# zhirui-gao/Curve-Gaussian

Hardware: AMD Instinct MI355X
Metric: Msplats rasterized/s (fwd+bwd) (higher is better)
Workload: dtype f32

## Files before the change

curve_gaussian_amd/csrc/render.hip:

```cpp
#include "kernels.h"
#include "p2_mfma.h"
#include "composite.h"

namespace cgs {

constexpr int BATCH = 256;
__device__ __forceinline__ float sat01(float x) { return __builtin_amdgcn_fmed3f(x, 0.f, 1.f); }
struct StepConsts {
    float big, cA;
};
__device__ __forceinline__ StepConsts step_consts() {
    StepConsts k;
    k.big = 0x1p100f;
    k.cA = -__uint_as_float(0x3b808080u) * 0x1p100f;
    asm volatile("" : "+v"(k.big), "+v"(k.cA));
    return k;
}
constexpr int SLOTS = 8;

struct BucketSort {
    const uint32_t* tile_count;
    const uint64_t* keys;
    uint32_t* point_list;
    uint2* ranges;
    uint32_t* total;
    uint32_t cap;
};

struct ViewEpilogue {
    float* color_clamped;
    float* dir_out;
    const float* wv;
};

constexpr int GROUP = 16;
#ifndef CGS_FWD3_WAVES
#define CGS_FWD3_WAVES 6
#endif
#ifndef CGS_FWD3_WAVES_GENERAL
#define CGS_FWD3_WAVES_GENERAL CGS_FWD3_WAVES
#endif
#ifndef CGS_FWD_FAST
#define CGS_FWD_FAST 1
#endif
#ifndef CGS_BWD3_WAVES
#define CGS_BWD3_WAVES 6
#endif
#ifndef CGS_BWD3_CAP
#define CGS_BWD3_CAP 104
#endif
constexpr int BWD_BATCH = 128;
static_assert(CGS_BWD3_CAP % 8 == 0 && CGS_BWD3_CAP <= BWD_BATCH, "CGS_BWD3_CAP: a multiple of SLOTS (8), at most BWD_BATCH");
constexpr uint32_t BWD_PAD_OFF = (BWD_BATCH + 1) * 16;
constexpr uint32_t PAD_OFF = (BATCH + 1) * 16;

template <bool GEO, bool SORT, bool UNIT = false, bool TAG = UNIT>
__global__ void __launch_bounds__(256, UNIT ? CGS_FWD3_WAVES : CGS_FWD3_WAVES_GENERAL) k_render_fwd3(const uint2* __restrict__ ranges,
                                                     const uint32_t* __restrict__ point_list, int W, int H, int grid_x,
                                                     const SplatRec* __restrict__ rec, float* __restrict__ final_T,
                                                     uint32_t* __restrict__ n_contrib, const float* __restrict__ bg_color,
                                                     float* __restrict__ out_color, float* __restrict__ out_invdepth,
                                                     float* __restrict__ out_all_map, BucketSort bs, ViewEpilogue epi) {
    constexpr bool IMAGE_ONLY = UNIT && !GEO;
    __shared__ float4 s_geo[BATCH + 2];
    __shared__ float4 s_at[BATCH + 2];
    __shared__ float4 s_c[GEO ? BATCH + 2 : 1];
    __shared__ uint64_t s_qmask[4][4];
    __shared__ __attribute__((aligned(16))) uint32_t s_list[4][BATCH + GROUP];
    __shared__ __attribute__((aligned(16))) uint32_t s_ord[SORT ? RANK_MAX + RANK_U : 1];
    __shared__ uint32_t s_si[SORT ? RANK_MAX : 1];
    __shared__ uint32_t s_hist[SORT ? RANK_NB : 1], s_start[SORT ? RANK_NB + 1 : 1], s_mm[8];
    if (threadIdx.x == 0) {
        s_geo[BATCH + 1] = make_float4(0.f, 0.f, 0.f, 0.f);
        s_at[BATCH + 1] = make_float4(0.f, 0.f, 0.f, L2_NEVER);
        if (GEO) s_c[GEO ? BATCH + 1 : 0] = make_float4(0.f, 0.f, 0.f, 0.f);
    }
    const TileGeom g = tile_geom(W, H, grid_x);
    const int lane = g.lane;
    const float X0 = (float)(g.tx * TILE), Y0 = (float)(g.ty * TILE);
    uint2 range;
    bool prestaged = false;
    if (SORT) {
        const uint32_t tid = threadIdx.x;
        const uint32_t base = g.tile * bs.cap;
        uint64_t key0 = ~0ull;
        if (CGS_FWD_FAST && tid < bs.cap) key0 = bs.keys[base + tid];
        const uint32_t cnt = bs.tile_count[g.tile];
        const uint32_t n = min(cnt, bs.cap);
        range = make_uint2(base, base + n);
        if (tid == 0) {
            bs.ranges[g.tile] = range;
            if (cnt) {
                uint32_t* part = bs.total + 4 + 2 * (g.tile % TOTAL_PARTS);
                atomicAdd(&part[0], n);
                atomicMax(&part[1], cnt);
                if (cnt > bs.cap) {
                    bs.total[2] = 1u;
                    atomicAdd(&bs.total[TOTAL_WORDS], 1u);
                }
            }
        }
        if (CGS_FWD_FAST && n > 0 && n <= (uint32_t)BATCH) {
            const bool has = tid < n;
            const uint32_t depth = has ? (uint32_t)(key0 >> 32) : ~0u;
            const uint32_t id = has ? (uint32_t)key0 : 0u;
            const SplatRec* r = rec + id;
            float4 ra = make_float4(0.f, 0.f, 1.f, 0.f), rb = make_float4(1.f, 0.f, 0.f, 0.f), rc = ra;
            float tau2 = -1.f;
            if (has) {
                ra = r->a;
                rb = r->b;
                if (GEO) rc = r->c;
                tau2 = r->d.z;
            }
            if (has) s_ord[tid] = depth;
            if (tid < 4u) s_ord[n + tid] = 0x7f800000u;
            s_si[tid] = 0u;
            __syncthreads();
            uint32_t lost = 0u;
            if (((uint32_t)__builtin_amdgcn_readfirstlane((int)tid) & ~63u) < n) {
                const uint32_t rk[1] = {rank_loop_f32(reinterpret_cast<const float*>(s_ord), n, __uint_as_float(depth))};
                if (has) {
                    float4 sa, sb;
                    stage_splat(ra, rb, sa, sb);
                    const uint32_t slot = rk[0] + 1u;
                    s_geo[slot] = sa;
                    s_at[slot] = make_float4(sb.z, sb.w, sb.x, __builtin_amdgcn_logf(sb.y));
                    if (GEO) s_c[GEO ? slot : 0] = UNIT ? make_float4(rc.x, rc.y, rc.z, sb.w) : rc;
                    const uint32_t qm = quadrant_mask(ra, rb, tau2, X0, Y0);
                    lost = atomicExch(&s_si[rk[0]], 0x100u | qm);
                    bs.point_list[base + rk[0]] = TAG ? (id | (qm << LIST_TAG_SHIFT)) : id;
                }
            }
            prestaged = !__syncthreads_or((int)lost);
        }
        if (n > 0 && !prestaged) {
            uint32_t rank[4], idx[4];
            tile_rank_sort<4>(bs.keys + base, n, RankScratch{s_ord, s_si, s_hist, s_start, s_mm}, rank, idx);
#pragma unroll
            for (int q = 0; q < 4; q++) {
                const uint32_t i = tid + 256u * q;
                if (i < n) {
                    s_ord[rank[q]] = idx[q];
                    if (!TAG || rank[q] >= (uint32_t)BATCH) bs.point_list[base + rank[q]] = idx[q];
                }
            }
            __syncthreads();
        }
    } else {
        range = ranges[g.tile];
    }
    const int total = (int)(range.y - range.x);
    const int rounds = (total + BATCH - 1) / BATCH;
    const StepConsts k = step_consts();
    float T_dead = 0.0f;
    float Tw = 1.0f;
    float cA = g.inside ? k.cA : -0x1p126f;
    uint32_t last_contributor = 0;
    float C = 0.f, Dacc = 0.f;
    float A0 = 0.f, A1 = 0.f, A2 = 0.f, A3 = 0.f;
    bool wave_done = ballot64(cA > -0x1p120f) == 0ull;
    const P2Frag pix = p2_pixel_operand(lane);
    const int row_splat = p2_row_splat(lane);
    const float hx = X0 + (float)((g.wave & 1) << 3) + 3.5f;
    const float hy = Y0 + (float)((g.wave >> 1) << 3) + 4.f * (float)p2_row_half(lane) + 1.5f;
    uint32_t* const list = s_list[g.wave];
    const char* const geo_bytes = reinterpret_cast<const char*>(s_geo);
    const char* const at_bytes = reinterpret_cast<const char*>(s_at);
    const char* const c_bytes = reinterpret_cast<const char*>(s_c);

    for (int i = 0; i < rounds; i++) {
        if (!prestaged) {
            if (!__syncthreads_or(!wave_done)) break;
            const int progress = i * BATCH + threadIdx.x;
            uint32_t qm = 0;
            if (progress < total) {
                const uint32_t id = SORT ? s_ord[progress] : point_list[range.x + progress];
                const SplatRec* r = rec + id;
                const float4 a = r->a, b = r->b;
                float4 sa, sb;
                stage_splat(a, b, sa, sb);
                s_geo[threadIdx.x + 1] = sa;
                s_at[threadIdx.x + 1] = make_float4(sb.z, sb.w, sb.x, __builtin_amdgcn_logf(sb.y));
                if (GEO) s_c[threadIdx.x + 1] = UNIT ? make_float4(r->c.x, r->c.y, r->c.z, sb.w) : r->c;
                qm = quadrant_mask(a, b, r->d.z, X0, Y0);
                if (TAG) const_cast<uint32_t*>(SORT ? bs.point_list : point_list)[range.x + progress] = id | (qm << LIST_TAG_SHIFT);
            }
#pragma unroll
            for (int q = 0; q < 4; q++) {
                const uint64_t bal = ballot64((qm >> q) & 1u);
                if (lane == 0) s_qmask[q][g.wave] = bal;
            }
            __syncthreads();
        }
        if (wave_done) continue;
        int n = 0;
#pragma unroll
        for (int c = 0; c < 4; c++) {
            const uint64_t m = prestaged ? ballot64((s_si[SORT ? c * 64 + lane : 0] >> g.wave) & 1u) : uniform64(s_qmask[g.wave][c]);
            if ((m >> lane) & 1ull) {
                const int pos = n + (int)__builtin_amdgcn_mbcnt_hi((uint32_t)(m >> 32), __builtin_amdgcn_mbcnt_lo((uint32_t)m, 0u));
                list[pos] = (uint32_t)((c * 64 + lane + 1) * 16);
            }
            n += __builtin_popcountll(m);
        }
        if (lane < GROUP) list[n + lane] = PAD_OFF;
        __builtin_amdgcn_fence(__ATOMIC_RELEASE, "wavefront");
        __builtin_amdgcn_wave_barrier();
        __builtin_amdgcn_fence(__ATOMIC_ACQUIRE, "wavefront");
        uint32_t last_off = 0;
        for (int g0 = 0; g0 < n; g0 += GROUP) {
            f32x16 P;
            {
                const uint32_t joff = list[g0 + row_splat];
                const float4 ge = *reinterpret_cast<const float4*>(geo_bytes + joff);
                const float2 cl = *reinterpret_cast<const float2*>(at_bytes + joff + 8);
                P = p2_mfma(p2_splat_operand(lane, ge.x, ge.y, ge.z, ge.w, cl.x, cl.y, hx, hy), pix);
            }
            const int cnt = min(GROUP, n - g0);
            uint4 w4 = make_uint4(0u, 0u, 0u, 0u);
#pragma unroll
            for (int s = 0; s < GROUP; s += 2) {
                if (s < cnt) {
                if ((s & 3) == 0) w4 = *reinterpret_cast<const uint4*>(list + g0 + s);
                const uint32_t j0 = (s & 2) ? w4.z : w4.x, j1 = (s & 2) ? w4.w : w4.y;
                float2 t0 = make_float2(0.f, 0.f), t1 = t0;
                if (!UNIT) {
                    t0 = *reinterpret_cast<const float2*>(at_bytes + j0);
                    t1 = *reinterpret_cast<const float2*>(at_bytes + j1);
                }
                float4 c0 = make_float4(0.f, 0.f, 0.f, 0.f), c1 = c0;
                if (GEO) {
                    c0 = *reinterpret_cast<const float4*>(c_bytes + j0);
                    c1 = *reinterpret_cast<const float4*>(c_bytes + j1);
                }
                const float al0 = fminf(0.99f, __builtin_amdgcn_exp2f(P[s]));
                const float al1 = fminf(0.99f, __builtin_amdgcn_exp2f(P[s + 1]));
                const float a0 = al0 * sat01(fmaf(al0, k.big, cA));
                const float a1 = al1 * sat01(fmaf(al1, k.big, cA));
                float wa = a0 * Tw;
                float T1 = fmaf(-Tw, a0, Tw);
                float wb = a1 * T1;
                float T2 = fmaf(-T1, a1, T1);
                if (__builtin_expect(ballot64(T2 < 0.0001f) != 0ull, 0)) {
                    const bool d0 = T1 < 0.0001f;
                    T_dead = d0 ? Tw : T_dead;
                    wa = d0 ? 0.f : wa;
                    T1 = d0 ? 1.0f : T1;
                    const float a1e = d0 ? 0.f : a1;
                    wb = a1e * T1;
                    T2 = fmaf(-T1, a1e, T1);
                    const bool d1 = T2 < 0.0001f;
                    T_dead = d1 ? T1 : T_dead;
                    wb = d1 ? 0.f : wb;
                    T2 = d1 ? 1.0f : T2;
                    cA = (d0 || d1) ? -0x1p126f : cA;
                    if (UNIT) last_off = d0 ? j0 : d1 ? j1 : last_off;
                }
                Tw = T2;
                if (!UNIT) C = fmaf(t0.x, wa, C);
                if (!IMAGE_ONLY) Dacc = fmaf(UNIT ? c0.w : t0.y, wa, Dacc);
                if (GEO) { A0 = fmaf(c0.x, wa, A0); A1 = fmaf(c0.y, wa, A1); A2 = fmaf(c0.z, wa, A2); if (!UNIT) A3 = fmaf(c0.w, wa, A3); }
                if (!UNIT) C = fmaf(t1.x, wb, C);
                if (!IMAGE_ONLY) Dacc = fmaf(UNIT ? c1.w : t1.y, wb, Dacc);
                if (GEO) { A0 = fmaf(c1.x, wb, A0); A1 = fmaf(c1.y, wb, A1); A2 = fmaf(c1.z, wb, A2); if (!UNIT) A3 = fmaf(c1.w, wb, A3); }
                if (!UNIT) {
                    last_off = max(min(last_off, j0), min(max(last_off, j0), __float_as_uint(wa)));
                    last_off = max(min(last_off, j1), min(max(last_off, j1), __float_as_uint(wb)));
                }
            }
            }
            if (ballot64(cA > -0x1p120f) == 0ull) {
                wave_done = true;
                break;
            }
        }
        if (last_off) last_contributor = (uint32_t)(i * BATCH) + (last_off >> 4) - (UNIT ? 1u : 0u);
    }
    const bool terminated = !(cA > -0x1p120f);
    if (UNIT && !terminated) last_contributor = (uint32_t)total;
    if (g.inside) {
        const size_t HW = (size_t)H * W;
        const float T = terminated ? T_dead : Tw;
        final_T[g.pix_id] = T;
        n_contrib[g.pix_id] = last_contributor | (terminated ? NCONTRIB_TERMINATED : 0u);
        if (UNIT) C = A3 = 1.f - T;
        const float Cout = C + T * bg_color[0];
        out_color[g.pix_id] = Cout;
        if (SORT && epi.color_clamped) epi.color_clamped[g.pix_id] = fminf(fmaxf(Cout, 0.f), 1.f);
        if (SORT && GEO && epi.dir_out) {
            const float* wv = epi.wv;
            epi.dir_out[g.pix_id] = A0 * wv[0] + A1 * wv[1] + A2 * wv[2];
            epi.dir_out[HW + g.pix_id] = A0 * wv[4] + A1 * wv[5] + A2 * wv[6];
            epi.dir_out[2 * HW + g.pix_id] = A0 * wv[8] + A1 * wv[9] + A2 * wv[10];
        }
        if (!IMAGE_ONLY) out_invdepth[g.pix_id] = Dacc;
        if (IMAGE_ONLY) {
        } else if (GEO) {
            out_all_map[g.pix_id] = A0;
            out_all_map[HW + g.pix_id] = A1;
            out_all_map[2 * HW + g.pix_id] = A2;
            out_all_map[3 * HW + g.pix_id] = A3;
        } else {
            out_all_map[g.pix_id] = 0.f;
            out_all_map[HW + g.pix_id] = 0.f;
            out_all_map[2 * HW + g.pix_id] = 0.f;
            out_all_map[3 * HW + g.pix_id] = 0.f;
        }
    }
}

__device__ __forceinline__ float rows_sum(float v) {
    const unsigned x = __float_as_uint(v);
    auto s16 = __builtin_amdgcn_permlane16_swap(x, x, false, false);
    const float t = __uint_as_float(s16[0]) + __uint_as_float(s16[1]);
    const unsigned y = __float_as_uint(t);
    auto s32 = __builtin_amdgcn_permlane32_swap(y, y, false, false);
    return __uint_as_float(s32[0]) + __uint_as_float(s32[1]);
}

constexpr int SSTRIDE = 80, LSTRIDE = 68;
__device__ __forceinline__ int slot_row(int q) { return 8 * q + 4 * (q >= 2) + 4 * (q >= 6); }
__device__ __forceinline__ int sum_field(int f) { return 8 * f + 4 * (f >= 4); }

template <bool GEO, bool INVD, bool COLG>
#ifndef CGS_BWD3_WAVES_GEO
#define CGS_BWD3_WAVES_GEO 3
#endif
#ifndef CGS_BWD3_WAVES_EXTRA
#define CGS_BWD3_WAVES_EXTRA 4
#endif
#ifndef CGS_BWD3_CAP_EXTRA
#define CGS_BWD3_CAP_EXTRA 96
#endif
#ifndef CGS_BWD3_CAP_GEO
#define CGS_BWD3_CAP_GEO 64
#endif
__global__ void __launch_bounds__(256, GEO ? CGS_BWD3_WAVES_GEO : (INVD || COLG) ? CGS_BWD3_WAVES_EXTRA : CGS_BWD3_WAVES) k_render_bwd3(
    const uint2* __restrict__ ranges, const uint32_t* __restrict__ point_list, int W, int H, int grid_x,
    const float* __restrict__ bg_color, const SplatRec* __restrict__ rec, const float* __restrict__ final_Ts,
    const uint32_t* __restrict__ n_contrib, const float* __restrict__ dL_dpixels,
    const float* __restrict__ dL_dout_invdepth, const float* __restrict__ dL_dout_all_map,
    float* __restrict__ grad_acc, int acc_stride, uint32_t id_mask, const uint32_t* __restrict__ nonunit_gate) {
    if (nonunit_gate && *nonunit_gate == 0u) return;
    constexpr bool EXTRA = COLG || INVD || GEO;
    constexpr bool MULTI = INVD || GEO;
    static_assert(!MULTI || COLG, "the instances with depth / all_map gradients also produce the colour gradient");
    constexpr int NF = GEO ? 12 : EXTRA ? 8 : 6;
    constexpr int NX = (COLG ? 1 : 0) + (INVD ? 1 : 0) + (GEO ? 4 : 0);
    constexpr int BB = BWD_BATCH, NC = BB / 64;
    constexpr int CAP = GEO ? CGS_BWD3_CAP_GEO : EXTRA ? CGS_BWD3_CAP_EXTRA : CGS_BWD3_CAP;
    static_assert(CAP % 8 == 0 && CAP <= BB, "CAP: a multiple of SLOTS (8), at most BWD_BATCH");
    __shared__ float4 s_geo[BB + 2];
    __shared__ float4 s_at[BB + 2];
    __shared__ float4 s_c[GEO ? BB + 2 : 1];
    __shared__ uint32_t s_id[INVD ? BB + 2 : 1];
    __shared__ uint64_t s_qmask[4][NC];
    __shared__ uint64_t s_tmask[4][NC];
    __shared__ __attribute__((aligned(16))) uint32_t s_list[4][BB + GROUP];
    __shared__ __attribute__((aligned(16))) float s_g[4][SLOTS * SSTRIDE];
    __shared__ __attribute__((aligned(16))) float s_w[EXTRA ? 4 : 1][EXTRA ? SLOTS * SSTRIDE : 1];
    __shared__ __attribute__((aligned(16))) float s_res[4][CAP * NF];
    __shared__ __attribute__((aligned(16))) float s_d[MULTI ? 4 : 1][MULTI ? NX : 1][64];
    const TileGeom g = tile_geom(W, H, grid_x);
    const int lane = g.lane;
    const float X0 = (float)(g.tx * TILE), Y0 = (float)(g.ty * TILE);
    const uint2 range = ranges[g.tile];
    const int total = (int)(range.y - range.x);
    if (total == 0) return;
    const int rounds = (total + BB - 1) / BB;
    const size_t HW = (size_t)H * W;
    const bool tagged = id_mask != 0xffffffffu;
    if (threadIdx.x == 0) {
        s_geo[BB + 1] = make_float4(0.f, 0.f, 0.f, 0.f);
        s_at[BB + 1] = make_float4(0.f, 0.f, 0.f, L2_NEVER);
        if (GEO) s_c[GEO ? BB + 1 : 0] = make_float4(0.f, 0.f, 0.f, 0.f);
        if (INVD) s_id[BB + 1] = 0u;
    }

    const float T_final = g.inside ? final_Ts[g.pix_id] : 0.f;
    float T = T_final;
    const uint32_t last_contributor = g.inside ? backward_cut(n_contrib[g.pix_id], (uint32_t)total) : 0u;
    uint32_t wave_last = last_contributor;
#pragma unroll
    for (int off = 32; off >= 1; off >>= 1) wave_last = max(wave_last, (uint32_t)__shfl_xor((int)wave_last, off, 64));
    wave_last = __builtin_amdgcn_readfirstlane(wave_last);

    float accum_rec = 0.f;
    float dL_dpixel = 0.f, dL_invd = 0.f, dm0 = 0.f, dm1 = 0.f, dm2 = 0.f, dm3 = 0.f;
    if (g.inside) {
        dL_dpixel = dL_dpixels[g.pix_id];
        if (INVD) dL_invd = dL_dout_invdepth[g.pix_id];
        if (GEO) {
            dm0 = dL_dout_all_map[g.pix_id];
            dm1 = dL_dout_all_map[HW + g.pix_id];
            dm2 = dL_dout_all_map[2 * HW + g.pix_id];
            dm3 = dL_dout_all_map[3 * HW + g.pix_id];
        }
    }
    const float nTf_bg = -T_final * (bg_color[0] * dL_dpixel);
    float Tp = T_final * dL_dpixel;
    uint32_t* const list = s_list[g.wave];
    const StepConsts k = step_consts();
    float* const sg = s_g[g.wave];
    float* const sw = s_w[EXTRA ? g.wave : 0];
    float* const res = s_res[g.wave];
    const char* const geo_bytes = reinterpret_cast<const char*>(s_geo);
    const char* const at_bytes = reinterpret_cast<const char*>(s_at);
    const char* const c_bytes = reinterpret_cast<const char*>(s_c);
    const P2Frag pix = p2_pixel_operand(lane);
    const int row_splat = p2_row_splat(lane);
    const float qx0 = (float)(g.tx * TILE + ((g.wave & 1) << 3));
    const float hx = qx0 + 3.5f;
    const float hy = Y0 + (float)((g.wave >> 1) << 3) + 4.f * (float)p2_row_half(lane) + 1.5f;
    const int sl = lane & (SLOTS - 1), q = lane >> 3;
    const int fs = lane >> 3, ff = lane & 7;
    const float qyr = (float)(g.ty * TILE + ((g.wave >> 1) << 3) + q);
    const int pix_off = slot_row(lane >> 3) + (lane & 7);
    if (MULTI) {
        const float mine[6] = {dL_dpixel, INVD ? dL_invd : dm0, INVD ? dm0 : dm1, INVD ? dm1 : dm2, INVD ? dm2 : dm3, dm3};
#pragma unroll
        for (int c = 0; c < NX; c++) s_d[MULTI ? g.wave : 0][MULTI ? c : 0][lane] = mine[c];
    }
    const float* const drow = &s_d[MULTI ? g.wave : 0][0][8 * q];

    for (int i = 0; i < rounds; i++) {
        if (i > 0) __syncthreads();
        const int progress = i * BB + threadIdx.x;
        uint32_t qm = 0;
        if (threadIdx.x < BB && progress < total) {
            const uint32_t ent = point_list[range.y - progress - 1];
            const uint32_t id = ent & id_mask;
            const SplatRec* r = rec + id;
            const float4 a = r->a, b = r->b;
            float4 sa, sb;
            stage_splat(a, b, sa, sb);
            if (INVD) s_id[threadIdx.x + 1] = id;
            s_geo[threadIdx.x + 1] = sa;
            s_at[threadIdx.x + 1] = make_float4(sb.z, INVD ? sb.w : __uint_as_float(id), sb.x, __builtin_amdgcn_logf(sb.y));
            if (GEO) s_c[threadIdx.x + 1] = r->c;
            qm = tagged ? (ent >> LIST_TAG_SHIFT) : quadrant_mask(a, b, r->d.z, X0, Y0);
        }
        if (g.wave < NC) {
#pragma unroll
            for (int qq = 0; qq < 4; qq++) {
                const uint64_t bal = ballot64((qm >> qq) & 1u);
                if (lane == 0) s_qmask[qq][g.wave] = bal;
            }
        }
        __syncthreads();
        const int first_J = total - (int)wave_last - i * BB;
        int n = 0;
#pragma unroll
        for (int c = 0; c < NC; c++) {
            uint64_t m = uniform64(s_qmask[g.wave][c]);
            const int lo = first_J - c * 64;
            if (lo >= 64) m = 0;
            else if (lo > 0) m &= ~((1ull << lo) - 1ull);
            if (lane == 0) s_tmask[g.wave][c] = m;
            if ((m >> lane) & 1ull) {
                const int pos = n + (int)__builtin_amdgcn_mbcnt_hi((uint32_t)(m >> 32), __builtin_amdgcn_mbcnt_lo((uint32_t)m, 0u));
                list[pos] = (uint32_t)((c * 64 + lane + 1) * 16);
            }
            n += __builtin_popcountll(m);
        }
        if (lane < GROUP) list[n + lane] = BWD_PAD_OFF;
        const int first_lane = total - (int)last_contributor - i * BB;
        const float jmin_f = (float)(16 * max(first_lane, 0));
        __builtin_amdgcn_fence(__ATOMIC_RELEASE, "wavefront");
        __builtin_amdgcn_wave_barrier();
        __builtin_amdgcn_fence(__ATOMIC_ACQUIRE, "wavefront");
        for (int g0 = 0; g0 < n; g0 += GROUP) {
            f32x16 P;
            {
                const uint32_t joff = list[g0 + row_splat];
                const float4 ge = *reinterpret_cast<const float4*>(geo_bytes + joff);
                const float2 cl = *reinterpret_cast<const float2*>(at_bytes + joff + 8);
                P = p2_mfma(p2_splat_operand(lane, ge.x, ge.y, ge.z, ge.w, cl.x, cl.y, hx, hy), pix);
            }
#pragma unroll
            for (int half = 0; half < 2; half++) {
                const int k0 = g0 + half * SLOTS;
                if (k0 < n) {
                    const uint4 wa4 = *reinterpret_cast<const uint4*>(list + k0);
                    const uint4 wb4 = *reinterpret_cast<const uint4*>(list + k0 + 4);
                    const uint32_t wv[SLOTS] = {wa4.x, wa4.y, wa4.z, wa4.w, wb4.x, wb4.y, wb4.z, wb4.w};
                    float2 ci[SLOTS];
                    float4 cm[GEO ? SLOTS : 1];
#pragma unroll
                    for (int u = 0; u < SLOTS; u++) {
                        if (MULTI) ci[u] = *reinterpret_cast<const float2*>(at_bytes + wv[u]);
                        else ci[u] = make_float2(*reinterpret_cast<const float*>(at_bytes + wv[u]), 0.f);
                        if (GEO) cm[GEO ? u : 0] = *reinterpret_cast<const float4*>(c_bytes + wv[u]);
                    }
#pragma unroll
                    for (int u = 0; u < SLOTS; u++) {
                        const float e = __builtin_amdgcn_exp2f(P[half * SLOTS + u]);
                        const float m = sat01(fmaf(e, k.big, k.cA)) * sat01((float)wv[u] - jmin_f);
                        const float alpha_u = e * m;
                        const float alpha = fminf(0.99f, alpha_u);
                        const float rcp_1ma = __builtin_amdgcn_rcpf(1.f - alpha);
                        float dL_dalpha, v_w = 0.f;
                        if (!MULTI) {
                            Tp = Tp * rcp_1ma;
                            const float d_c = ci[u].x - accum_rec;
                            accum_rec = fmaf(alpha, d_c, accum_rec);
                            if (COLG) v_w = alpha * Tp;
                            dL_dalpha = fmaf(nTf_bg, rcp_1ma, d_c * Tp);
                        } else {
                            T = T * rcp_1ma;
                            float chat = ci[u].x * dL_dpixel;
                            if (INVD) chat = fmaf(ci[u].y, dL_invd, chat);
                            if (GEO) {
                                const float4 c4 = cm[GEO ? u : 0];
                                chat = fmaf(c4.x, dm0, chat); chat = fmaf(c4.y, dm1, chat);
                                chat = fmaf(c4.z, dm2, chat); chat = fmaf(c4.w, dm3, chat);
                            }
                            const float d_c = chat - accum_rec;
                            accum_rec = fmaf(alpha, d_c, accum_rec);
                            v_w = alpha * T;
                            dL_dalpha = fmaf(nTf_bg, rcp_1ma, d_c * T);
                        }
                        sg[u * SSTRIDE + pix_off] = alpha_u * dL_dalpha;
                        if (EXTRA) sw[u * SSTRIDE + pix_off] = v_w;
                    }
                    __builtin_amdgcn_fence(__ATOMIC_RELEASE, "wavefront");
                    __builtin_amdgcn_wave_barrier();
                    __builtin_amdgcn_fence(__ATOMIC_ACQUIRE, "wavefront");
                    float Sg, Sx, Sy, Sxx, Sxy, Syy;
                    float E[EXTRA ? NX : 1];
                    {
                        const uint32_t joff = list[k0 + sl];
                        const float2 cxy = *reinterpret_cast<const float2*>(geo_bytes + joff);
                        const float dx0 = cxy.x - qx0, dyr = cxy.y - qyr;
                        const float4 g0v = *reinterpret_cast<const float4*>(sg + sl * SSTRIDE + slot_row(q));
                        const float4 g1v = *reinterpret_cast<const float4*>(sg + sl * SSTRIDE + slot_row(q) + 4);
                        float M0 = g0v.x + g0v.y, M1 = g0v.y, M2 = g0v.y;
                        M0 += g0v.z; M1 = fmaf(g0v.z, 2.f, M1); M2 = fmaf(g0v.z, 4.f, M2);
                        M0 += g0v.w; M1 = fmaf(g0v.w, 3.f, M1); M2 = fmaf(g0v.w, 9.f, M2);
                        M0 += g1v.x; M1 = fmaf(g1v.x, 4.f, M1); M2 = fmaf(g1v.x, 16.f, M2);
                        M0 += g1v.y; M1 = fmaf(g1v.y, 5.f, M1); M2 = fmaf(g1v.y, 25.f, M2);
                        M0 += g1v.z; M1 = fmaf(g1v.z, 6.f, M1); M2 = fmaf(g1v.z, 36.f, M2);
                        M0 += g1v.w; M1 = fmaf(g1v.w, 7.f, M1); M2 = fmaf(g1v.w, 49.f, M2);
                        const float Rx = fmaf(dx0, M0, -M1);
                        const float Rxx = fmaf(dx0, Rx - M1, M2);
                        Sg = M0; Sx = Rx; Sxx = Rxx;
                        Sy = dyr * M0; Sxy = dyr * Rx; Syy = (dyr * dyr) * M0;
                        if (EXTRA) {
                            const float4 w0v = *reinterpret_cast<const float4*>(sw + sl * SSTRIDE + slot_row(q));
                            const float4 w1v = *reinterpret_cast<const float4*>(sw + sl * SSTRIDE + slot_row(q) + 4);
                            if (!MULTI) {
                                E[0] = ((w0v.x + w0v.y) + (w0v.z + w0v.w)) + ((w1v.x + w1v.y) + (w1v.z + w1v.w));
                            } else {
#pragma unroll
                                for (int c = 0; c < NX; c++) {
                                    const float4 d0 = *reinterpret_cast<const float4*>(drow + 64 * c);
                                    const float4 d1 = *reinterpret_cast<const float4*>(drow + 64 * c + 4);
                                    float e = w0v.x * d0.x;
                                    e = fmaf(w0v.y, d0.y, e); e = fmaf(w0v.z, d0.z, e); e = fmaf(w0v.w, d0.w, e);
                                    e = fmaf(w1v.x, d1.x, e); e = fmaf(w1v.y, d1.y, e); e = fmaf(w1v.z, d1.z, e);
                                    E[c] = fmaf(w1v.w, d1.w, e);
                                }
                            }
                        }
                    }
                    __builtin_amdgcn_fence(__ATOMIC_RELEASE, "wavefront");
                    __builtin_amdgcn_wave_barrier();
                    __builtin_amdgcn_fence(__ATOMIC_ACQUIRE, "wavefront");
                    {
                        float* rp = sg + sl * LSTRIDE + q;
                        rp[sum_field(0)] = Sg; rp[sum_field(1)] = Sx; rp[sum_field(2)] = Sy;
                        rp[sum_field(3)] = Sxx; rp[sum_field(4)] = Sxy; rp[sum_field(5)] = Syy;
                        if (EXTRA) {
                            rp[sum_field(ACC_COL)] = E[0];
                            rp[sum_field(ACC_INVD)] = INVD ? E[1] : 0.f;
                            if (GEO) {
                                float* xp = sw + sl * LSTRIDE + q;
                                constexpr int M0I = INVD ? 2 : 1;
                                xp[sum_field(0)] = E[GEO ? M0I : 0]; xp[sum_field(1)] = E[GEO ? M0I + 1 : 0];
                                xp[sum_field(2)] = E[GEO ? M0I + 2 : 0]; xp[sum_field(3)] = E[GEO ? M0I + 3 : 0];
                            }
                        }
                    }
                    __builtin_amdgcn_fence(__ATOMIC_RELEASE, "wavefront");
                    __builtin_amdgcn_wave_barrier();
                    __builtin_amdgcn_fence(__ATOMIC_ACQUIRE, "wavefront");
                    {
                        float v = 0.f, v2 = 0.f;
                        if (ff < (EXTRA ? 8 : 6)) {
                            const float4 r0 = *reinterpret_cast<const float4*>(sg + fs * LSTRIDE + sum_field(ff));
                            const float4 r1 = *reinterpret_cast<const float4*>(sg + fs * LSTRIDE + sum_field(ff) + 4);
                            v = ((r0.x + r0.y) + (r0.z + r0.w)) + ((r1.x + r1.y) + (r1.z + r1.w));
                        }
                        if (GEO && ff < 4) {
                            const float4 r0 = *reinterpret_cast<const float4*>(sw + fs * LSTRIDE + sum_field(ff));
                            const float4 r1 = *reinterpret_cast<const float4*>(sw + fs * LSTRIDE + sum_field(ff) + 4);
                            v2 = ((r0.x + r0.y) + (r0.z + r0.w)) + ((r1.x + r1.y) + (r1.z + r1.w));
                        }
                        if (CAP >= BB || k0 + SLOTS <= CAP) {
                            if (ff < (NF < 8 ? NF : 8)) res[(k0 + fs) * NF + ff] = v;
                            if (GEO && ff < 4) res[(k0 + fs) * NF + 8 + ff] = v2;
                        } else {
                            const uint32_t joff = list[k0 + fs];
                            const uint32_t id = INVD ? *reinterpret_cast<const uint32_t*>(reinterpret_cast<const char*>(s_id) + (joff >> 2))
                                                     : __float_as_uint(*reinterpret_cast<const float*>(at_bytes + joff + 4));
                            if (v != 0.f) atomicAdd(grad_acc + (size_t)id * acc_stride + ff, v);
                            if (GEO && v2 != 0.f) atomicAdd(grad_acc + (size_t)id * acc_stride + 8 + ff, v2);
                        }
                    }
                    __builtin_amdgcn_fence(__ATOMIC_RELEASE, "wavefront");
                    __builtin_amdgcn_wave_barrier();
                    __builtin_amdgcn_fence(__ATOMIC_ACQUIRE, "wavefront");
                }
            }
        }
        __syncthreads();
        const int nb = min(BB, total - i * BB);
        uint64_t tm[4][NC];
        int base[4][NC];
#pragma unroll
        for (int w = 0; w < 4; w++) {
            int acc = 0;
#pragma unroll
            for (int c = 0; c < NC; c++) { tm[w][c] = s_tmask[w][c]; base[w][c] = acc; acc += __builtin_popcountll(tm[w][c]); }
        }
        constexpr int FL = NF > 8 ? 16 : 8;
        constexpr int EPP = 256 / FL;
        const int f = (int)(threadIdx.x & (FL - 1));
#pragma unroll
        for (int c = 0; c < NC; c++) {
#pragma unroll
            for (int h = 0; h < 64 / EPP; h++) {
                const int bit = h * EPP + (int)(threadIdx.x / FL), e = c * 64 + bit;
                if (e < nb && f < NF) {
                    float v = 0.f;
                    bool any = false;
#pragma unroll
                    for (int w = 0; w < 4; w++) {
                        const uint64_t m = tm[w][c];
                        const int pos = base[w][c] + __builtin_popcountll(m & ((1ull << bit) - 1ull));
                        if (((m >> bit) & 1ull) && pos < CAP) { v += s_res[w][pos * NF + f]; any = true; }
                    }
                    if (any && v != 0.f) {
                        const uint32_t id = INVD ? s_id[e + 1] : __float_as_uint(s_at[e + 1].y);
                        atomicAdd(grad_acc + (size_t)id * acc_stride + f, v);
                    }
                }
            }
        }
    }
}

#define CGS_FWD3(G, S, U, T, R, PL, BS)                                                                               \
    hipLaunchKernelGGL((k_render_fwd3<G, S, U, T>), dim3(tiles), dim3(256), 0, s, R, PL, W, H, grid_x, rec, final_T,  \
                       n_contrib, bg_color, out_color, out_invdepth, out_all_map, BS, epi)
void launch_render_fwd(hipStream_t s, bool geo, int tiles, const uint2* ranges, const uint32_t* point_list, int W,
                       int H, int grid_x, const SplatRec* rec, float* final_T, uint32_t* n_contrib,
                       const float* bg_color, float* out_color, float* out_invdepth, float* out_all_map, bool unit, bool tag) {
    ProfScope p("render_fwd", s);
    const ViewEpilogue epi{nullptr, nullptr, nullptr};
    if (geo && unit) CGS_FWD3(true, false, true, true, ranges, point_list, BucketSort{});
    else if (unit) CGS_FWD3(false, false, true, true, ranges, point_list, BucketSort{});
    else if (geo && tag) CGS_FWD3(true, false, false, true, ranges, point_list, BucketSort{});
    else if (tag) CGS_FWD3(false, false, false, true, ranges, point_list, BucketSort{});
    else if (geo) CGS_FWD3(true, false, false, false, ranges, point_list, BucketSort{});
    else CGS_FWD3(false, false, false, false, ranges, point_list, BucketSort{});
}
bool render_fwd_can_sort(uint32_t cap) { return cap <= RANK_MAX; }
void launch_render_fwd_sorting(hipStream_t s, bool geo, int tiles, const uint32_t* tile_count, const uint64_t* keys,
                               uint32_t cap, uint2* ranges, uint32_t* total, uint32_t* point_list, int W, int H,
                               int grid_x, const SplatRec* rec, float* final_T, uint32_t* n_contrib,
                               const float* bg_color, float* out_color, float* out_invdepth, float* out_all_map, bool unit,
                               bool tag, float* color_clamped, float* dir_out, const float* wv) {
    ProfScope p("render_fwd", s);
    const BucketSort bs{tile_count, keys, point_list, ranges, total, cap};
    const ViewEpilogue epi{color_clamped, geo ? dir_out : nullptr, wv};
    const uint2* no_ranges = nullptr;
    const uint32_t* no_list = nullptr;
    if (geo && unit) CGS_FWD3(true, true, true, true, no_ranges, no_list, bs);
    else if (unit) CGS_FWD3(false, true, true, true, no_ranges, no_list, bs);
    else if (geo && tag) CGS_FWD3(true, true, false, true, no_ranges, no_list, bs);
    else if (tag) CGS_FWD3(false, true, false, true, no_ranges, no_list, bs);
    else if (geo) CGS_FWD3(true, true, false, false, no_ranges, no_list, bs);
    else CGS_FWD3(false, true, false, false, no_ranges, no_list, bs);
}
#undef CGS_FWD3
void launch_render_bwd(hipStream_t s, bool geo, bool invd, bool colg, int tiles, const uint2* ranges,
                       const uint32_t* point_list, int W, int H, int grid_x, const float* bg_color,
                       const SplatRec* rec, const float* final_Ts, const uint32_t* n_contrib, const float* dL_dpixels,
                       const float* dL_dout_invdepth, const float* dL_dout_all_map, float* grad_acc, int acc_stride,
                       uint32_t id_mask, const uint32_t* nonunit_gate) {
    ProfScope p("render_bwd", s);
#define CGS_BWD(G, I, C)                                                                                         \
    hipLaunchKernelGGL((k_render_bwd3<G, I, C>), dim3(tiles), dim3(256), 0, s, ranges, point_list, W, H, grid_x, \
                       bg_color, rec, final_Ts, n_contrib, dL_dpixels, dL_dout_invdepth, dL_dout_all_map, grad_acc, acc_stride, id_mask, nonunit_gate)
    if (geo && invd) CGS_BWD(true, true, true);
    else if (geo) CGS_BWD(true, false, true);
    else if (invd) CGS_BWD(false, true, true);
    else if (colg) CGS_BWD(false, false, true);
    else CGS_BWD(false, false, false);
#undef CGS_BWD
}

}
```

curve_gaussian_amd/csrc/render_unit_bwd.hip:

```cpp
#include "kernels.h"
#include "composite.h"
#include "p2_mfma.h"

namespace cgs {

#ifndef CGS_UBWD_WAVES
#define CGS_UBWD_WAVES 6
#endif
constexpr int UB = 256;
constexpr int CH = 32;
constexpr int KROW = 36;
constexpr uint32_t ENT_PAD = (uint32_t)UB;

__device__ __forceinline__ float dpp_wave_shr1(float v) {
    return __builtin_bit_cast(float, __builtin_amdgcn_update_dpp(0, __builtin_bit_cast(int, v), 0x138, 0xF, 0xF, true));
}
__device__ __forceinline__ float swap32_sum(float v) {
    const unsigned x = __float_as_uint(v);
    auto s = __builtin_amdgcn_permlane32_swap(x, x, false, false);
    return __uint_as_float(s[0]) + __uint_as_float(s[1]);
}
__device__ __forceinline__ float swap32_pair_sum(float lo, float hi) {
    auto s = __builtin_amdgcn_permlane32_swap(__float_as_uint(lo), __float_as_uint(hi), false, false);
    return __uint_as_float(s[0]) + __uint_as_float(s[1]);
}
__device__ __forceinline__ void wave_lds_fence() {
    __builtin_amdgcn_fence(__ATOMIC_RELEASE, "wavefront");
    __builtin_amdgcn_wave_barrier();
    __builtin_amdgcn_fence(__ATOMIC_ACQUIRE, "wavefront");
}

__device__ __forceinline__ P2Frag ub_pack(float t0, float t1, float t2) {
    uint32_t a0, a1, a2, b0, b1, b2, c0, c1, c2;
    split3(t0, a0, a1, a2);
    split3(t1, b0, b1, b2);
    split3(t2, c0, c1, c2);
    P2Frag f;
    f.k0 = u32x4{pack2(a0, a1), pack2(b0, b1), pack2(b2, c0), pack2(c1, c2)};
    f.k1 = u32x4{a2 >> 16, 0u, 0u, 0u};
    return f;
}
__device__ __forceinline__ P2Frag ub_pixel_operand(int lane, int block) {
    const int m = lane & 31;
    const float u = (float)((m & 3) + 4 * ((m >> 3) & 1)) - 3.5f;
    const float v = (float)(4 * block + ((m >> 2) & 1) + 2 * (m >> 4)) - 3.5f;
    const bool hi_half = lane >= 32;
    const float m0 = hi_half ? u : 1.0f, m1 = hi_half ? u * u : v, m2 = hi_half ? v * v : u * v;
    const uint32_t b0 = __float_as_uint(m0), b1 = __float_as_uint(m1), b2 = __float_as_uint(m2);
    P2Frag f;
    f.k0 = u32x4{pack2(b0, b0), pack2(b1, b1), pack2(b1, b2), pack2(b2, b2)};
    f.k1 = u32x4{b0 >> 16, 0u, 0u, 0u};
    return f;
}

struct WalkConsts { float one, floor01, amin, ramin; };
__device__ __forceinline__ WalkConsts walk_consts() {
    WalkConsts k;
    k.one = 1.0f;
    k.floor01 = 1.0f - 0.99f;
    k.amin = ALPHA_MIN;
    k.ramin = 255.0f;
    asm volatile("" : "+v"(k.one), "+v"(k.floor01), "+v"(k.amin), "+v"(k.ramin));
    return k;
}

template <bool SLOW, bool LEAN>
__device__ __forceinline__ void masked_add(float& s, float v, float x, float thr, uint32_t pos, uint32_t cut) {
#define CGS_UB_CMPX_E "v_cmpx_nlt_f32_e32 vcc, %[x], %[thr]\n\t"
#define CGS_UB_CMPX_R "v_cmpx_ngt_f32_e32 vcc, %[x], %[thr]\n\t"
#define CGS_UB_TAIL "v_add_f32_e32 %[s], %[s], %[v]\n\ts_mov_b64 exec, -1"
    if (SLOW) {
        if (LEAN)
            asm volatile(CGS_UB_CMPX_R "v_cmpx_lt_u32_e32 vcc, %[pos], %[cut]\n\t" CGS_UB_TAIL
                         : [s] "+v"(s) : [x] "v"(x), [thr] "v"(thr), [pos] "v"(pos), [cut] "v"(cut), [v] "v"(v) : "vcc");
        else
            asm volatile(CGS_UB_CMPX_E "v_cmpx_lt_u32_e32 vcc, %[pos], %[cut]\n\t" CGS_UB_TAIL
                         : [s] "+v"(s) : [x] "v"(x), [thr] "v"(thr), [pos] "v"(pos), [cut] "v"(cut), [v] "v"(v) : "vcc");
    } else {
        if (LEAN) asm volatile(CGS_UB_CMPX_R CGS_UB_TAIL : [s] "+v"(s) : [x] "v"(x), [thr] "v"(thr), [v] "v"(v) : "vcc");
        else asm volatile(CGS_UB_CMPX_E CGS_UB_TAIL : [s] "+v"(s) : [x] "v"(x), [thr] "v"(thr), [v] "v"(v) : "vcc");
    }
#undef CGS_UB_CMPX_E
#undef CGS_UB_CMPX_R
#undef CGS_UB_TAIL
}

template <bool SLOW, bool LEAN>
__device__ __forceinline__ void ub_walk_row(const f32x16& nP, int r0, const float* __restrict__ krow, const uint32_t* __restrict__ lrow,
                                            uint32_t pos, const WalkConsts& k, float& R0, float& R1, float& R2) {
    float s = 0.f, u = 0.f, w = 0.f;
#pragma unroll
    for (int rr = 1; rr >= 0; rr--) {
        const float4 K4 = *reinterpret_cast<const float4*>(krow + r0 + 4 * rr);
        uint4 L4 = make_uint4(0u, 0u, 0u, 0u);
        if (SLOW) L4 = *reinterpret_cast<const uint4*>(lrow + r0 + 4 * rr);
        const float Kv[4] = {K4.x, K4.y, K4.z, K4.w};
        const uint32_t Lv[4] = {L4.x, L4.y, L4.z, L4.w};
#pragma unroll
        for (int t = 3; t >= 0; t--) {
            if (LEAN) {
                const float E = __builtin_amdgcn_exp2f(nP[r0 + 4 * rr + t]);
                const float v = __builtin_amdgcn_rcpf(fmaf(E, Kv[t], -Kv[t]));
                masked_add<SLOW, true>(s, v, E, k.ramin, pos, Lv[t]);
            } else {
                const float e = __builtin_amdgcn_exp2f(-nP[r0 + 4 * rr + t]);
                const float om = fmaxf(k.one - e, k.floor01);
                const float v = (e * Kv[t]) * __builtin_amdgcn_rcpf(om);
                masked_add<SLOW, false>(s, v, e, k.amin, pos, Lv[t]);
            }
            if (4 * rr + t > 0) { u += s; w += u; }
        }
    }
    R0 = s;
    R1 = u;
    R2 = (w + w) - u;
}

template <int STRIDE, bool GATED>
__global__ void __launch_bounds__(256, CGS_UBWD_WAVES) k_render_bwd_unit(
    const uint2* __restrict__ ranges, const uint32_t* __restrict__ point_list, int W, int H, int grid_x,
    const float* __restrict__ bg_color, const SplatRec* __restrict__ rec, const float* __restrict__ final_Ts,
    const uint32_t* __restrict__ n_contrib, const float* __restrict__ dL_dpixels, float* __restrict__ grad_acc,
    const uint32_t* __restrict__ nonunit_gate, const float* __restrict__ clamp_raw) {
    if (GATED && *nonunit_gate != 0u) return;
    __shared__ float4 s_geo[UB + 1];
    __shared__ float4 s_at[UB + 1];
    __shared__ uint16_t s_list[UB * 4 + CH];
    __shared__ __attribute__((aligned(16))) float s_K[8 * KROW];
    __shared__ __attribute__((aligned(16))) float s_Kinv[8 * KROW];
    __shared__ __attribute__((aligned(16))) uint32_t s_last[8 * KROW];
    __shared__ uint32_t s_wcount[4];
    __shared__ uint32_t s_qlast[8];
    __shared__ __attribute__((aligned(16))) float s_out[4][CH][8];

    const TileGeom g = tile_geom(W, H, grid_x);
    const int lane = g.lane;
    const uint2 range = ranges[g.tile];
    const int total = (int)(range.y - range.x);
    if (total == 0) return;
    const float X0 = (float)(g.tx * TILE), Y0 = (float)(g.ty * TILE);

    {
        float K = 0.f;
        uint32_t last = 0u;
        if (g.inside) {
            const float T_final = final_Ts[g.pix_id];
            float dL = dL_dpixels[g.pix_id];
            if (clamp_raw) {
                const float x = clamp_raw[g.pix_id];
                dL = (x >= 0.f && x <= 1.f) ? dL : 0.f;
            }
            K = T_final * dL - T_final * (bg_color[0] * dL);
            last = backward_cut(n_contrib[g.pix_id], (uint32_t)total);
        }
        const int x = lane & 7, y = lane >> 3;
        const int b = y >> 2, yy = y & 3, hh = yy & 1, r = x + 8 * (yy >> 1);
        const int idx = (g.wave * 2 + hh) * KROW + b * 16 + r;
        s_K[idx] = K;
        s_Kinv[idx] = fabsf(K) > 1e-30f ? __builtin_amdgcn_rcpf(K) : 1e30f;
        s_last[idx] = last;
        uint32_t mx = last, mn = g.inside ? last : 0xffffffffu;
#pragma unroll
        for (int off = 32; off >= 1; off >>= 1) {
            mx = max(mx, (uint32_t)__shfl_xor((int)mx, off, 64));
            mn = min(mn, (uint32_t)__shfl_xor((int)mn, off, 64));
        }
        if (lane == 0) {
            s_qlast[g.wave] = mx;
            s_qlast[4 + g.wave] = mn;
        }
        if (threadIdx.x == 0) {
            s_geo[UB] = make_float4(0.f, 0.f, 0.f, 0.f);
            s_at[UB] = make_float4(0.f, L2_NEVER, 0.f, 0.f);
        }
    }
    __syncthreads();
    uint32_t qmax[4], qmin[4];
#pragma unroll
    for (int q = 0; q < 4; q++) {
        qmax[q] = __builtin_amdgcn_readfirstlane(s_qlast[q]);
        qmin[q] = __builtin_amdgcn_readfirstlane(s_qlast[4 + q]);
    }
    const int nb = min(total, (int)max(max(qmax[0], qmax[1]), max(qmax[2], qmax[3])));
    const int rounds = (nb + UB - 1) / UB;

    const P2Frag pix0 = ub_pixel_operand(lane, 0), pix1 = ub_pixel_operand(lane, 1);
    const int n = lane & 31, hh = lane >> 5;
    const WalkConsts wk = walk_consts();
    float* const outw = &s_out[g.wave][0][0];

    for (int i = 0; i < rounds; i++) {
        if (i > 0) __syncthreads();
        const int pos = i * UB + (int)threadIdx.x;
        uint32_t qm = 0, cutm = 0;
        if (pos < nb) {
            const uint32_t tagged = point_list[range.x + pos];
            const uint32_t id = tagged & LIST_ID_MASK;
            const SplatRec* r = rec + id;
            const float4 a = r->a, b = r->b;
            float4 sa, sb;
            stage_splat(a, b, sa, sb);
            s_geo[threadIdx.x] = sa;
            s_at[threadIdx.x] = make_float4(sb.x, __builtin_amdgcn_logf(sb.y), __uint_as_float(id), 0.f);
            qm = tagged >> LIST_TAG_SHIFT;
#pragma unroll
            for (int q = 0; q < 4; q++) {
                if ((uint32_t)pos >= qmax[q]) qm &= ~(1u << q);
                if ((uint32_t)pos >= qmin[q]) cutm |= 1u << q;
            }
        }
        uint32_t before = 0, wave_pairs = 0;
#pragma unroll
        for (int q = 0; q < 4; q++) {
            const uint64_t bal = ballot64((qm >> q) & 1u);
            before += __builtin_amdgcn_mbcnt_hi((uint32_t)(bal >> 32), __builtin_amdgcn_mbcnt_lo((uint32_t)bal, 0u));
            wave_pairs += (uint32_t)__builtin_popcountll(bal);
        }
        if (lane == 0) s_wcount[g.wave] = wave_pairs;
        __syncthreads();
        uint32_t n_pairs = 0;
        {
            uint32_t base = 0;
#pragma unroll
            for (int w = 0; w < 4; w++) {
                const uint32_t c = s_wcount[w];
                base += w < g.wave ? c : 0u;
                n_pairs += c;
            }
            if (qm) {
                const uint32_t cnt = (uint32_t)__builtin_popcount(qm);
                uint32_t p = base + before, k = 0;
#pragma unroll
                for (int q = 0; q < 4; q++)
                    if ((qm >> q) & 1u) {
                        s_list[p + k] = (uint16_t)(threadIdx.x | ((uint32_t)q << 9) | (k << 11) | ((cnt - 1u) << 13) |
                                                   (((cutm >> q) & 1u) << 15));
                        k++;
                    }
            }
            if (threadIdx.x < CH) s_list[n_pairs + threadIdx.x] = (uint16_t)ENT_PAD;
        }
        __syncthreads();
        const int nch = (int)((n_pairs + CH - 1) / CH);
        for (int c = g.wave; c < nch; c += 4) {
            const uint32_t ent = s_list[c * CH + n];
            const uint32_t J = ent & 511u, q = (ent >> 9) & 3u, run_k = (ent >> 11) & 3u, run_last = (ent >> 13) & 3u;
            const bool valid = (uint32_t)(c * CH + n) < n_pairs;
            const float4 ge = s_geo[J];
            const float4 at = s_at[J];
            const float qox = X0 + (float)((q & 1u) << 3), qoy = Y0 + (float)((q >> 1) << 3);
            P2Frag bf;
            {
                const float dxc = ge.x - (qox + 3.5f), dyc = ge.y - (qoy + 3.5f);
                const float A2 = ge.z, B2 = ge.w, C2 = at.x;
                const float c0 = dxc * (A2 * dxc + B2 * dyc) + C2 * dyc * dyc + at.y;
                const float cu = -(2.f * A2 * dxc + B2 * dyc);
                const float cv = -(B2 * dxc + 2.f * C2 * dyc);
                bf = ub_pack(hh ? -cu : -c0, hh ? -A2 : -cv, hh ? -C2 : -B2);
            }
            const uint32_t lpos = (uint32_t)(i * UB) + J;
            const bool slow = ballot64((ent >> 15) != 0u) != 0ull;
            const bool lean = ballot64(at.y >= -0.02f) == 0ull;
            const float* const krow = (lean ? s_Kinv : s_K) + (q * 2u + (uint32_t)hh) * KROW;
            const uint32_t* const lrow = s_last + (q * 2u + (uint32_t)hh) * KROW;
            float N00 = 0.f, X1 = 0.f, X2 = 0.f, Y1 = 0.f, Y2 = 0.f, XY = 0.f;
#pragma unroll
            for (int b = 0; b < 2; b++) {
                f32x16 P = {};
                const P2Frag& px = b ? pix1 : pix0;
                P = __builtin_amdgcn_mfma_f32_32x32x16_bf16(__builtin_bit_cast(bf16x8, px.k0), __builtin_bit_cast(bf16x8, bf.k0), P, 0, 0, 0);
                P = __builtin_amdgcn_mfma_f32_32x32x16_bf16(__builtin_bit_cast(bf16x8, pix0.k1), __builtin_bit_cast(bf16x8, bf.k1), P, 0, 0, 0);
                float r0, r1, r2;
                const int variant = (slow ? 2 : 0) + (lean ? 1 : 0);
#define CGS_UB_ROW(R)                                                                                        \
    if (variant == 3) ub_walk_row<true, true>(P, R, krow + 16 * b, lrow + 16 * b, lpos, wk, r0, r1, r2);        \
    else if (variant == 2) ub_walk_row<true, false>(P, R, krow + 16 * b, lrow + 16 * b, lpos, wk, r0, r1, r2);  \
    else if (variant == 1) ub_walk_row<false, true>(P, R, krow + 16 * b, lrow + 16 * b, lpos, wk, r0, r1, r2);  \
    else if (variant == 0) ub_walk_row<false, false>(P, R, krow + 16 * b, lrow + 16 * b, lpos, wk, r0, r1, r2)
                CGS_UB_ROW(0);
                N00 += r0; X1 += r1; X2 += r2;
                if (b) { Y1 = fmaf(2.f, r0, Y1); Y2 = fmaf(4.f, r0, Y2); XY = fmaf(2.f, r1, XY); }
                CGS_UB_ROW(8);
#undef CGS_UB_ROW
                N00 += r0; X1 += r1; X2 += r2;
                const float j = (float)(2 * b + 1);
                Y1 = fmaf(j, r0, Y1); Y2 = fmaf(j * j, r0, Y2); XY = fmaf(j, r1, XY);
            }
            const float Dx = ge.x - qox, Dy = ge.y - (qoy + (float)hh);
            float Sg = N00;
            float Sx = fmaf(Dx, N00, -X1);
            float Sy = fmaf(Dy, N00, -2.f * Y1);
            float Sxx = fmaf(Dx, Sx - X1, X2);
            float Syy = fmaf(Dy, Sy - 2.f * Y1, 4.f * Y2);
            float Sxy = fmaf(Dx, Sy, fmaf(-Dy, X1, 2.f * XY));
            float v0 = swap32_pair_sum(Sg, Sxx), v1 = swap32_pair_sum(Sx, Sxy), v2 = swap32_pair_sum(Sy, Syy);
            const uint32_t k_eff = min(run_k, (uint32_t)n);
            {
                const float t0 = dpp_wave_shr1(v0), t1 = dpp_wave_shr1(v1), t2 = dpp_wave_shr1(v2);
                if (k_eff >= 1u) { v0 += t0; v1 += t1; v2 += t2; }
                const float u0 = dpp_wave_shr1(dpp_wave_shr1(v0)), u1 = dpp_wave_shr1(dpp_wave_shr1(v1)), u2 = dpp_wave_shr1(dpp_wave_shr1(v2));
                if (k_eff >= 2u) { v0 += u0; v1 += u1; v2 += u2; }
            }
            const bool leader = valid && (run_k == run_last || n == CH - 1);
            const uint32_t lmask = (uint32_t)ballot64(leader);
            const uint32_t slot = (uint32_t)__builtin_popcount(lmask & ((1u << n) - 1u));
            const int n_lead = __builtin_popcount(lmask);
            if (leader) {
                float* o = outw + slot * 8u + (hh ? 3 : 0);
                o[0] = v0; o[1] = v1; o[2] = v2;
                if (!hh) outw[slot * 8u + 6u] = at.z;
            }
            wave_lds_fence();
            for (int e0 = 0; e0 < n_lead; e0 += 8) {
                const int e = e0 + (lane >> 3), f = lane & 7;
                if (e < n_lead && f < 6) {
                    const float v = outw[e * 8 + f];
                    const uint32_t id = __float_as_uint(outw[e * 8 + 6]);
                    if (v != 0.f) atomicAdd(grad_acc + (size_t)id * STRIDE + f, v);
                }
            }
            wave_lds_fence();
        }
    }
}

void launch_render_bwd_unit(hipStream_t s, int tiles, const uint2* ranges, const uint32_t* point_list, int W, int H,
                            int grid_x, const float* bg_color, const SplatRec* rec, const float* final_Ts,
                            const uint32_t* n_contrib, const float* dL_dpixels, float* grad_acc, int acc_stride,
                            const uint32_t* nonunit_gate, const float* clamp_raw) {
    ProfScope p(nonunit_gate ? "render_bwd_unit_gated" : "render_bwd", s);
    if (acc_stride == ACC_STRIDE_VIEW && !nonunit_gate)
        hipLaunchKernelGGL((k_render_bwd_unit<ACC_STRIDE_VIEW, false>), dim3(tiles), dim3(256), 0, s, ranges, point_list, W, H,
                           grid_x, bg_color, rec, final_Ts, n_contrib, dL_dpixels, grad_acc, nullptr, clamp_raw);
    else if (acc_stride == ACC_STRIDE && nonunit_gate)
        hipLaunchKernelGGL((k_render_bwd_unit<ACC_STRIDE, true>), dim3(tiles), dim3(256), 0, s, ranges, point_list, W, H, grid_x,
                           bg_color, rec, final_Ts, n_contrib, dL_dpixels, grad_acc, nonunit_gate, clamp_raw);
    else
        set_error("launch_render_bwd_unit: unsupported (stride %d, gate %p) combination", acc_stride, (const void*)nonunit_gate);
}

}
```

Measured before the change: 815.3.

## Stage MFMA pixel operands in LDS and raise occupancy to seven waves

The per-lane pixel MFMA operand fragments are now precomputed once into shared memory and reloaded right before each MFMA, instead of being held in registers for the whole kernel. The k1 fragment is rebuilt from a shift of k0. The launch bounds for forward and unit backward go from 6 to 7 waves per SIMD, and s_si/s_fmask are aliased into existing shared buffers to hold down LDS growth. The aim is to lower VGPR pressure so more waves can be resident, at the cost of extra LDS reads inside the hot loop and possible spills under the tighter register budget.

After: 850.2, median of 6. +4.3%, better.

```diff
diff --git a/curve_gaussian_amd/csrc/render.hip b/curve_gaussian_amd/csrc/render.hip
--- a/curve_gaussian_amd/csrc/render.hip
+++ b/curve_gaussian_amd/csrc/render.hip
@@ -35,7 +35,7 @@
 
 constexpr int GROUP = 16;
 #ifndef CGS_FWD3_WAVES
-#define CGS_FWD3_WAVES 6
+#define CGS_FWD3_WAVES 7
 #endif
 #ifndef CGS_FWD3_WAVES_GENERAL
 #define CGS_FWD3_WAVES_GENERAL CGS_FWD3_WAVES
@@ -68,8 +68,13 @@
     __shared__ uint64_t s_qmask[4][4];
     __shared__ __attribute__((aligned(16))) uint32_t s_list[4][BATCH + GROUP];
     __shared__ __attribute__((aligned(16))) uint32_t s_ord[SORT ? RANK_MAX + RANK_U : 1];
-    __shared__ uint32_t s_si[SORT ? RANK_MAX : 1];
     __shared__ uint32_t s_hist[SORT ? RANK_NB : 1], s_start[SORT ? RANK_NB + 1 : 1], s_mm[8];
+    static_assert(!SORT || sizeof(s_list) >= RANK_MAX * sizeof(uint32_t), "s_si lives in s_list");
+    static_assert(RANK_MAX / 2 >= BATCH + RANK_U && RANK_MAX / 2 + BATCH <= RANK_MAX, "s_fmask lives in the upper half of s_ord");
+    uint32_t* const s_si = &s_list[0][0];
+    uint32_t* const s_fmask = s_ord + (SORT ? RANK_MAX / 2 : 0);
+    __shared__ __attribute__((aligned(16))) u32x4 s_pix[64];
+    if (threadIdx.x < 64) s_pix[threadIdx.x] = p2_pixel_operand((int)threadIdx.x).k0;
     if (threadIdx.x == 0) {
         s_geo[BATCH + 1] = make_float4(0.f, 0.f, 0.f, 0.f);
         s_at[BATCH + 1] = make_float4(0.f, 0.f, 0.f, L2_NEVER);
@@ -115,7 +120,7 @@
             }
             if (has) s_ord[tid] = depth;
             if (tid < 4u) s_ord[n + tid] = 0x7f800000u;
-            s_si[tid] = 0u;
+            s_fmask[tid] = 0u;
             __syncthreads();
             uint32_t lost = 0u;
             if (((uint32_t)__builtin_amdgcn_readfirstlane((int)tid) & ~63u) < n) {
@@ -128,7 +133,7 @@
                     s_at[slot] = make_float4(sb.z, sb.w, sb.x, __builtin_amdgcn_logf(sb.y));
                     if (GEO) s_c[GEO ? slot : 0] = UNIT ? make_float4(rc.x, rc.y, rc.z, sb.w) : rc;
                     const uint32_t qm = quadrant_mask(ra, rb, tau2, X0, Y0);
-                    lost = atomicExch(&s_si[rk[0]], 0x100u | qm);
+                    lost = atomicExch(&s_fmask[rk[0]], 0x100u | qm);
                     bs.point_list[base + rk[0]] = TAG ? (id | (qm << LIST_TAG_SHIFT)) : id;
                 }
             }
@@ -160,11 +165,11 @@
     float C = 0.f, Dacc = 0.f;
     float A0 = 0.f, A1 = 0.f, A2 = 0.f, A3 = 0.f;
     bool wave_done = ballot64(cA > -0x1p120f) == 0ull;
-    const P2Frag pix = p2_pixel_operand(lane);
+    const int wave = __builtin_amdgcn_readfirstlane(g.wave);
     const int row_splat = p2_row_splat(lane);
-    const float hx = X0 + (float)((g.wave & 1) << 3) + 3.5f;
-    const float hy = Y0 + (float)((g.wave >> 1) << 3) + 4.f * (float)p2_row_half(lane) + 1.5f;
-    uint32_t* const list = s_list[g.wave];
+    const float hx = X0 + (float)((wave & 1) << 3) + 3.5f;
+    const float hy = Y0 + (float)((wave >> 1) << 3) + 4.f * (float)p2_row_half(lane) + 1.5f;
+    uint32_t* const list = s_list[wave];
     const char* const geo_bytes = reinterpret_cast<const char*>(s_geo);
     const char* const at_bytes = reinterpret_cast<const char*>(s_at);
     const char* const c_bytes = reinterpret_cast<const char*>(s_c);
@@ -189,7 +194,7 @@
 #pragma unroll
             for (int q = 0; q < 4; q++) {
                 const uint64_t bal = ballot64((qm >> q) & 1u);
-                if (lane == 0) s_qmask[q][g.wave] = bal;
+                if (lane == 0) s_qmask[q][wave] = bal;
             }
             __syncthreads();
         }
@@ -197,7 +202,7 @@
         int n = 0;
 #pragma unroll
         for (int c = 0; c < 4; c++) {
-            const uint64_t m = prestaged ? ballot64((s_si[SORT ? c * 64 + lane : 0] >> g.wave) & 1u) : uniform64(s_qmask[g.wave][c]);
+            const uint64_t m = prestaged ? ballot64((s_fmask[SORT ? c * 64 + lane : 0] >> wave) & 1u) : uniform64(s_qmask[wave][c]);
             if ((m >> lane) & 1ull) {
                 const int pos = n + (int)__builtin_amdgcn_mbcnt_hi((uint32_t)(m >> 32), __builtin_amdgcn_mbcnt_lo((uint32_t)m, 0u));
                 list[pos] = (uint32_t)((c * 64 + lane + 1) * 16);
@@ -215,6 +220,11 @@
                 const uint32_t joff = list[g0 + row_splat];
                 const float4 ge = *reinterpret_cast<const float4*>(geo_bytes + joff);
                 const float2 cl = *reinterpret_cast<const float2*>(at_bytes + joff + 8);
+                uint32_t pix_off = (uint32_t)lane * 16u;
+                asm volatile("" : "+v"(pix_off));
+                P2Frag pix;
+                pix.k0 = *reinterpret_cast<const u32x4*>(reinterpret_cast<const char*>(s_pix) + pix_off);
+                pix.k1 = u32x4{pix.k0.w >> 16, 0u, 0u, 0u};
                 P = p2_mfma(p2_splat_operand(lane, ge.x, ge.y, ge.z, ge.w, cl.x, cl.y, hx, hy), pix);
             }
             const int cnt = min(GROUP, n - g0);
diff --git a/curve_gaussian_amd/csrc/render_unit_bwd.hip b/curve_gaussian_amd/csrc/render_unit_bwd.hip
--- a/curve_gaussian_amd/csrc/render_unit_bwd.hip
+++ b/curve_gaussian_amd/csrc/render_unit_bwd.hip
@@ -5,7 +5,7 @@
 namespace cgs {
 
 #ifndef CGS_UBWD_WAVES
-#define CGS_UBWD_WAVES 6
+#define CGS_UBWD_WAVES 7
 #endif
 constexpr int UB = 256;
 constexpr int CH = 32;
@@ -132,6 +132,7 @@
     __shared__ uint32_t s_wcount[4];
     __shared__ uint32_t s_qlast[8];
     __shared__ __attribute__((aligned(16))) float s_out[4][CH][8];
+    __shared__ __attribute__((aligned(16))) u32x4 s_pix[2][64];
 
     const TileGeom g = tile_geom(W, H, grid_x);
     const int lane = g.lane;
@@ -169,6 +170,10 @@
             s_qlast[g.wave] = mx;
             s_qlast[4 + g.wave] = mn;
         }
+        if (threadIdx.x < 64) {
+            s_pix[0][threadIdx.x] = ub_pixel_operand((int)threadIdx.x, 0).k0;
+            s_pix[1][threadIdx.x] = ub_pixel_operand((int)threadIdx.x, 1).k0;
+        }
         if (threadIdx.x == 0) {
             s_geo[UB] = make_float4(0.f, 0.f, 0.f, 0.f);
             s_at[UB] = make_float4(0.f, L2_NEVER, 0.f, 0.f);
@@ -184,7 +189,6 @@
     const int nb = min(total, (int)max(max(qmax[0], qmax[1]), max(qmax[2], qmax[3])));
     const int rounds = (nb + UB - 1) / UB;
 
-    const P2Frag pix0 = ub_pixel_operand(lane, 0), pix1 = ub_pixel_operand(lane, 1);
     const int n = lane & 31, hh = lane >> 5;
     const WalkConsts wk = walk_consts();
     float* const outw = &s_out[g.wave][0][0];
@@ -267,9 +271,12 @@
 #pragma unroll
             for (int b = 0; b < 2; b++) {
                 f32x16 P = {};
-                const P2Frag& px = b ? pix1 : pix0;
-                P = __builtin_amdgcn_mfma_f32_32x32x16_bf16(__builtin_bit_cast(bf16x8, px.k0), __builtin_bit_cast(bf16x8, bf.k0), P, 0, 0, 0);
-                P = __builtin_amdgcn_mfma_f32_32x32x16_bf16(__builtin_bit_cast(bf16x8, pix0.k1), __builtin_bit_cast(bf16x8, bf.k1), P, 0, 0, 0);
+                uint32_t pix_off = (uint32_t)lane * 16u;
+                asm volatile("" : "+v"(pix_off));
+                const u32x4 pk0 = *reinterpret_cast<const u32x4*>(reinterpret_cast<const char*>(s_pix[b]) + pix_off);
+                const u32x4 pk1 = u32x4{pk0.x >> 16, 0u, 0u, 0u};
+                P = __builtin_amdgcn_mfma_f32_32x32x16_bf16(__builtin_bit_cast(bf16x8, pk0), __builtin_bit_cast(bf16x8, bf.k0), P, 0, 0, 0);
+                P = __builtin_amdgcn_mfma_f32_32x32x16_bf16(__builtin_bit_cast(bf16x8, pk1), __builtin_bit_cast(bf16x8, bf.k1), P, 0, 0, 0);
                 float r0, r1, r2;
                 const int variant = (slow ? 2 : 0) + (lean ? 1 : 0);
 #define CGS_UB_ROW(R)                                                                                        \
```
